# url-kaist/Quatro

Measured on NVIDIA H100. Metric: registrations/sec (64-ring pair), higher is better.
Workload: dtype f32 (front end, match, graph filter) / f64 (graph boundary, GNC, COTE)

## Files before the change

### quatro_b200/csrc/frontend.cu

```cuda
#include <cub/device/device_radix_sort.cuh>
#include <type_traits>

#include "fpfh_math.cuh"
#include "handle.cuh"

namespace qb {

size_t sort_temp_bytes(int max_items) {
  size_t bytes = 0;
  cub::DeviceRadixSort::SortPairs(nullptr, bytes, (const uint64_t*)nullptr, (uint64_t*)nullptr, (const uint32_t*)nullptr,
                                  (uint32_t*)nullptr, max_items, 0, 64, (cudaStream_t)0);
  return bytes;
}

int sort_pairs(Lane* h, int n_items, int end_bit) {
  if (n_items <= 0) return QB200_OK;
  size_t bytes = h->cub_bytes;
  QB_CUDA_TRY(h, cub::DeviceRadixSort::SortPairs(h->cub_temp.get(), bytes, h->key_a.get(), h->key_b.get(), h->val_a.get(), h->val_b.get(), n_items, 0, end_bit,
                                                 h->stream));
  h->launches += 1 + (end_bit + 7) / 8;
  return QB200_OK;
}

static int clog2(int n) {
  int b = 0;
  while ((1 << b) < n) ++b;
  return b;
}


__global__ void __launch_bounds__(256) voxel_bbox_kernel(const float4* const* __restrict__ cloud_ptr, const int* __restrict__ cloud_n,
                                                         const CloudFront* __restrict__ front, int* __restrict__ bbox,
                                                         int* __restrict__ n_valid, int* __restrict__ chunk_cnt) {
  const int cloud = blockIdx.y;
  const int n = cloud_n[cloud];
  const int skip_flagged = front[cloud].skip_flagged;
  const float4* __restrict__ pts = cloud_ptr[cloud];
  int mn0 = INT_MAX, mn1 = INT_MAX, mn2 = INT_MAX, mx0 = INT_MIN, mx1 = INT_MIN, mx2 = INT_MIN, cnt = 0;
  constexpr int kInFlight = 8;
  __shared__ int s_cc[kVsChunks];
  if (threadIdx.x < kVsChunks) s_cc[threadIdx.x] = 0;
  __syncthreads();
  const int cs = vox_chunk_size(n);
  const int per_cta = kVsChunks / gridDim.x;
  for (int cl = 0; cl < per_cta; ++cl) {
    const int ch = blockIdx.x * per_cta + cl;
    const int c0 = ch * cs, c1 = min(n, c0 + cs);
    int ccnt = 0;
    for (int i0 = c0 + threadIdx.x; i0 < c1; i0 += kInFlight * 256) {
      float4 pp[kInFlight];
#pragma unroll
      for (int j = 0; j < kInFlight; ++j) pp[j] = i0 + j * 256 < c1 ? __ldg(pts + i0 + j * 256) : make_float4(NAN, NAN, NAN, 0.f);
#pragma unroll
      for (int j = 0; j < kInFlight; ++j) {
        const float4 p = pp[j];
        if (i0 + j * 256 >= c1 || !raw_point_kept(p, skip_flagged)) continue;
        const int ox = float_ordered(p.x), oy = float_ordered(p.y), oz = float_ordered(p.z);
        mn0 = min(mn0, ox); mn1 = min(mn1, oy); mn2 = min(mn2, oz);
        mx0 = max(mx0, ox); mx1 = max(mx1, oy); mx2 = max(mx2, oz);
        ++ccnt;
      }
    }
    cnt += ccnt;
    ccnt = __reduce_add_sync(0xffffffffu, ccnt);
    if (lane_id() == 0 && ccnt) atomicAdd(&s_cc[ch], ccnt);
  }
  __syncthreads();
  if ((int)threadIdx.x < per_cta) chunk_cnt[cloud * kVsChunks + blockIdx.x * per_cta + threadIdx.x] = s_cc[blockIdx.x * per_cta + threadIdx.x];
#pragma unroll
  for (int o = 16; o > 0; o >>= 1) {
    mn0 = min(mn0, __shfl_xor_sync(0xffffffffu, mn0, o)); mn1 = min(mn1, __shfl_xor_sync(0xffffffffu, mn1, o));
    mn2 = min(mn2, __shfl_xor_sync(0xffffffffu, mn2, o)); mx0 = max(mx0, __shfl_xor_sync(0xffffffffu, mx0, o));
    mx1 = max(mx1, __shfl_xor_sync(0xffffffffu, mx1, o)); mx2 = max(mx2, __shfl_xor_sync(0xffffffffu, mx2, o));
    cnt += __shfl_xor_sync(0xffffffffu, cnt, o);
  }
  __shared__ int s_red[7];
  if (threadIdx.x == 0) { s_red[0] = s_red[1] = s_red[2] = INT_MAX; s_red[3] = s_red[4] = s_red[5] = INT_MIN; s_red[6] = 0; }
  __syncthreads();
  if (lane_id() == 0 && cnt) {
    atomicMin(&s_red[0], mn0); atomicMin(&s_red[1], mn1); atomicMin(&s_red[2], mn2);
    atomicMax(&s_red[3], mx0); atomicMax(&s_red[4], mx1); atomicMax(&s_red[5], mx2);
    atomicAdd(&s_red[6], cnt);
  }
  __syncthreads();
  if (threadIdx.x == 0 && s_red[6]) {
    int* b = bbox + cloud * 6;
    atomicMin(b + 0, s_red[0]); atomicMin(b + 1, s_red[1]); atomicMin(b + 2, s_red[2]);
    atomicMax(b + 3, s_red[3]); atomicMax(b + 4, s_red[4]); atomicMax(b + 5, s_red[5]);
    atomicAdd(n_valid + cloud, s_red[6]);
  }
}

__global__ void __launch_bounds__(1024) run_heads_kernel(int mode, const uint64_t* keys, const uint64_t* keys_b, const int* __restrict__ seg_off,
                                                         int V, int key_shift, const CloudFront* __restrict__ front, const int* __restrict__ bbox,
                                                         const int* __restrict__ n_valid_in, int* __restrict__ starts,
                                                         uint64_t* __restrict__ cell_keys, int* __restrict__ n_out, int* __restrict__ n_valid_out,
                                                         int* __restrict__ cloud_status, int* __restrict__ digits_out) {
  __shared__ int sm[33];
  __shared__ int s_overflow, s_valid;
  const int cloud = blockIdx.x;
  const int off = mode == 0 ? seg_off[cloud] : cloud * V;
  const int n = mode == 0 ? n_valid_in[cloud] : V;
  const int digits = mode == 0 ? vox_digits(bbox + cloud * 6, n, front[cloud].inv_leaf) : 0;
  if (digits & 1) keys = keys_b;
  if (threadIdx.x == 0) {
    s_overflow = digits < 0 ? 1 : 0;
    s_valid = 0;
    if (digits_out) digits_out[cloud] = digits;
  }
  __syncthreads();
  if (s_overflow) {
    if (threadIdx.x == 0) {
      n_out[cloud] = 0;
      cloud_status[cloud] = QB200_ERR_VOXEL_OVERFLOW;
      starts[(size_t)cloud * (V + 1)] = 0;
    }
    return;
  }
  int carry = 0;
  constexpr int kPer = 4;
  for (int base = 0; base < n; base += kPer * blockDim.x) {
    const int p0 = base + kPer * threadIdx.x;
    uint64_t k[kPer];
    bool valid[kPer];
    int head[kPer], nh = 0, nv = 0;
    uint64_t kprev = (p0 > 0 && p0 < n) ? keys[off + p0 - 1] >> key_shift : 0;
#pragma unroll
    for (int j = 0; j < kPer; ++j) {
      const int p = p0 + j;
      k[j] = 0; valid[j] = false; head[j] = 0;
      if (p < n) {
        k[j] = keys[off + p] >> key_shift;
        valid[j] = mode == 0 ? (k[j] & kVoxMask) != kVoxInvalid : (k[j] & kCellMask) != kCellInvalid;
        head[j] = (valid[j] && (p == 0 || k[j] != kprev)) ? 1 : 0;
        kprev = k[j];
      }
      nh += head[j]; nv += valid[j] ? 1 : 0;
    }
    int both;
    const int exb = block_excl_scan(nh | (nv << 16), sm, &both);
    int rank = carry + (exb & 0xFFFF);
    const int tot = both & 0xFFFF, vtot = both >> 16;
#pragma unroll
    for (int j = 0; j < kPer; ++j) {
      if (head[j]) {
        if (rank <= V) {
          starts[(size_t)cloud * (V + 1) + rank] = p0 + j;
          if (mode == 1 && rank < V) cell_keys[(size_t)cloud * V + rank] = k[j] & kCellMask;
        }
        ++rank;
      }
    }
    carry += tot;
    if (threadIdx.x == 0) s_valid += vtot;
  }
  if (threadIdx.x == 0) {
    const int valid_total = s_valid;
    int nv = carry;
    if (nv > V) {
      nv = V;
      cloud_status[cloud] = QB200_CAPACITY_EXCEEDED;
    } else {
      starts[(size_t)cloud * (V + 1) + nv] = valid_total;
    }
    n_out[cloud] = nv;
    if (n_valid_out) n_valid_out[cloud] = valid_total;
  }
}

__global__ void __launch_bounds__(128) voxel_centroid_kernel(const float4* const* __restrict__ cloud_ptr, const int* __restrict__ raw_off,
                                                             const uint64_t* sorted_keys, const uint64_t* keys_b, const int* __restrict__ vox_digits,
                                                             uint64_t idx_mask,
                                                             const int* __restrict__ starts, const int* __restrict__ n_vox, int V,
                                                             float4* __restrict__ vox_pts) {
  const int cloud = blockIdx.y;
  const int r = blockIdx.x * blockDim.x + threadIdx.x;
  if (r >= n_vox[cloud]) return;
  const uint64_t* __restrict__ keys = ((vox_digits[cloud] & 1) ? keys_b : sorted_keys) + raw_off[cloud];
  const float4* __restrict__ pts = cloud_ptr[cloud];
  const int a = starts[(size_t)cloud * (V + 1) + r], b = starts[(size_t)cloud * (V + 1) + r + 1];
  float sx = 0.f, sy = 0.f, sz = 0.f;
  int t = a;
  for (; t + 4 <= b; t += 4) {
    const uint64_t k0 = keys[t], k1 = keys[t + 1], k2 = keys[t + 2], k3 = keys[t + 3];
    const float4 p0 = __ldg(pts + (k0 & idx_mask)), p1 = __ldg(pts + (k1 & idx_mask)), p2 = __ldg(pts + (k2 & idx_mask)),
                 p3 = __ldg(pts + (k3 & idx_mask));
    sx += p0.x; sy += p0.y; sz += p0.z;
    sx += p1.x; sy += p1.y; sz += p1.z;
    sx += p2.x; sy += p2.y; sz += p2.z;
    sx += p3.x; sy += p3.y; sz += p3.z;
  }
  for (; t < b; ++t) {
    const float4 p = __ldg(pts + (keys[t] & idx_mask));
    sx += p.x; sy += p.y; sz += p.z;
  }
  const float cnt = (float)(b - a);
  vox_pts[(size_t)cloud * V + r] = make_float4(sx / cnt, sy / cnt, sz / cnt, 1.0f);
}

__global__ void __launch_bounds__(256) lattice_keys_kernel(const float4* __restrict__ pts, const int* __restrict__ n_pts, int V,
                                                           const CloudFront* __restrict__ front, uint64_t* __restrict__ keys,
                                                           uint32_t* __restrict__ vals) {
  const int cloud = blockIdx.y;
  const int r = blockIdx.x * blockDim.x + threadIdx.x;
  if (r >= V) return;
  uint64_t cell = kCellInvalid;
  if (r < n_pts[cloud]) {
    const float inv_cell = front[cloud].inv_cell;
    const float4 p = pts[(size_t)cloud * V + r];
    if (isfinite(p.x) && isfinite(p.y) && isfinite(p.z)) {
      const int ci = (int)floorf(p.x * inv_cell), cj = (int)floorf(p.y * inv_cell), ck = (int)floorf(p.z * inv_cell);
      if (cell_ok(ci, cj, ck)) cell = cell_key(ci, cj, ck);
    }
  }
  keys[(size_t)cloud * V + r] = ((uint64_t)cloud << kCloudShift) | cell;
  vals[(size_t)cloud * V + r] = (uint32_t)r;
}

struct LatticeView {
  const float4* pts;
  const uint64_t* ckeys;
  const int* cstart;
  const uint32_t* order;
  int n_cells;
  float inv;
};

template <class R2, class F>
__device__ __forceinline__ void walk_cells(const LatticeView& L, const float4 pq, const R2& r2_src, int c0, int c1, F&& f) {
  if (c0 >= c1) return;
  const float r2 = r2_src;
  const int t1 = L.cstart[c1];
  for (int t = L.cstart[c0]; t < t1; t += 4) {
    int p[4];
    float4 pp[4];
#pragma unroll
    for (int e = 0; e < 4; ++e) p[e] = t + e < t1 ? (int)L.order[t + e] : -1;
#pragma unroll
    for (int e = 0; e < 4; ++e) pp[e] = p[e] >= 0 ? L.pts[p[e]] : make_float4(0.f, 0.f, 0.f, 0.f);
#pragma unroll
    for (int e = 0; e < 4; ++e) {
      if (p[e] < 0) continue;
      const float dx = pq.x - pp[e].x, dy = pq.y - pp[e].y, dz = pq.z - pp[e].z;
      const float d2 = (dx * dx + dy * dy) + dz * dz;
      if (d2 < r2) f(p[e], d2, pp[e]);
    }
  }
}

template <bool kLockstep = true, class R2, class F>
__device__ __forceinline__ void for_each_neighbor(const LatticeView& L, const float4 pq, int m, const R2& r2, F&& f) {
  if (!(isfinite(pq.x) && isfinite(pq.y) && isfinite(pq.z))) return;
  const int ci = (int)floorf(pq.x * L.inv), cj = (int)floorf(pq.y * L.inv), ck = (int)floorf(pq.z * L.inv);
  if (!cell_ok(ci, cj, ck)) return;
  const int ilo = max(ci - m, -kOffIJ), ihi = min(ci + m, kOffIJ - 2);
  if (kLockstep && m == 1) {
    uint64_t lo[9], hi[9];
    int a[9], b[9], e[9];
#pragma unroll
    for (int r = 0; r < 9; ++r) {
      const int k = ck + r / 3 - 1, j = cj + r % 3 - 1;
      const bool ok = !(k < -kOffK || k >= kOffK - 1 || j < -kOffIJ || j >= kOffIJ - 1);
      lo[r] = ok ? cell_key(ilo, j, k) : 1;
      hi[r] = ok ? cell_key(ihi, j, k) : 0;
      a[r] = 0; b[r] = ok ? L.n_cells : 0;
      e[r] = 0;
    }
    const int steps = 33 - __clz(L.n_cells | 1);
    for (int s = 0; s < steps; ++s) {
#pragma unroll
      for (int r = 0; r < 9; ++r) {
        if (a[r] < b[r]) {
          const int mid = (a[r] + b[r]) >> 1;
          if (L.ckeys[mid] < lo[r]) a[r] = mid + 1; else b[r] = mid;
        }
      }
    }
#pragma unroll
    for (int r = 0; r < 9; ++r) {
      int c = a[r];
#pragma unroll
      for (int q = 0; q < 3; ++q)
        if (c < L.n_cells && hi[r] >= lo[r] && L.ckeys[c] <= hi[r]) ++c;
      e[r] = c;
    }
#pragma unroll
    for (int r = 0; r < 9; ++r) walk_cells(L, pq, r2, a[r], e[r], f);
    return;
  }
  for (int dk = -m; dk <= m; ++dk) {
    const int k = ck + dk;
    if (k < -kOffK || k >= kOffK - 1) continue;
    for (int dj = -m; dj <= m; ++dj) {
      const int j = cj + dj;
      if (j < -kOffIJ || j >= kOffIJ - 1) continue;
      const uint64_t lo = cell_key(ilo, j, k), hi = cell_key(ihi, j, k);
      int a = 0, b = L.n_cells;
      while (a < b) {
        const int mid = (a + b) >> 1;
        if (L.ckeys[mid] < lo) a = mid + 1; else b = mid;
      }
      int c = a;
      while (c < L.n_cells && L.ckeys[c] <= hi) ++c;
      walk_cells(L, pq, r2, a, c, f);
    }
  }
}

__device__ __forceinline__ LatticeView make_view(int cloud, int V, const float4* pts, const uint64_t* cell_key, const int* cell_start,
                                                 const uint32_t* order, const int* n_cells, float inv) {
  LatticeView L;
  L.pts = pts + (size_t)cloud * V;
  L.ckeys = cell_key + (size_t)cloud * V;
  L.cstart = cell_start + (size_t)cloud * (V + 1);
  L.order = order + (size_t)cloud * V;
  L.n_cells = n_cells[cloud];
  L.inv = inv;
  return L;
}

constexpr int kNbrThreads = 128;
constexpr int kNbrCap = 32;

struct WalkPos {
  int row = 0;
  int t = -1;
};

__device__ __forceinline__ int walk_chunk(const LatticeView& L, const float4 pq, int m, float r2, WalkPos& pos,
                                          uint32_t (*nbr)[kNbrThreads]) {
  const int w = 2 * m + 1;
  if (!(isfinite(pq.x) && isfinite(pq.y) && isfinite(pq.z))) { pos.row = w * w; return 0; }
  const int ci = (int)floorf(pq.x * L.inv), cj = (int)floorf(pq.y * L.inv), ck = (int)floorf(pq.z * L.inv);
  if (!cell_ok(ci, cj, ck)) { pos.row = w * w; return 0; }
  const int ilo = max(ci - m, -kOffIJ), ihi = min(ci + m, kOffIJ - 2);
  int n = 0;
  for (; pos.row < w * w; ++pos.row, pos.t = -1) {
    const int k = ck + pos.row / w - m, j = cj + pos.row % w - m;
    if (k < -kOffK || k >= kOffK - 1 || j < -kOffIJ || j >= kOffIJ - 1) continue;
    const uint64_t lo = cell_key(ilo, j, k), hi = cell_key(ihi, j, k);
    int a = 0, b = L.n_cells;
    while (a < b) {
      const int mid = (a + b) >> 1;
      if (L.ckeys[mid] < lo) a = mid + 1; else b = mid;
    }
    int c = a;
    while (c < L.n_cells && L.ckeys[c] <= hi) ++c;
    if (a >= c) continue;
    const int t1 = L.cstart[c];
    for (int t = pos.t >= 0 ? pos.t : L.cstart[a]; t < t1; ++t) {
      const int p = (int)L.order[t];
      const float4 pp = L.pts[p];
      const float dx = pq.x - pp.x, dy = pq.y - pp.y, dz = pq.z - pp.z;
      const float d2 = (dx * dx + dy * dy) + dz * dz;
      if (!(d2 < r2)) continue;
      if (n == kNbrCap) { pos.t = t; return n; }
      nbr[n++][threadIdx.x] = (uint32_t)p;
    }
  }
  return n;
}

__global__ void __launch_bounds__(kNbrThreads) nbr_list_kernel(const float4* __restrict__ pts, const int* __restrict__ n_pts, int V,
                                                               const uint64_t* __restrict__ cell_key, const int* __restrict__ cell_start,
                                                               const uint32_t* __restrict__ order, const int* __restrict__ n_cells,
                                                               const CloudFront* __restrict__ front, uint32_t* __restrict__ nbr_list,
                                                               int* __restrict__ nbr_cnt) {
  volatile __shared__ float s_r2;
  const int cloud = blockIdx.y;
  if (threadIdx.x == 0) s_r2 = front[cloud].rf2;
  __syncthreads();
  const int q = blockIdx.x * blockDim.x + threadIdx.x;
  if (q >= n_pts[cloud]) return;
  const int m = front[cloud].mf;
  const LatticeView L = make_view(cloud, V, pts, cell_key, cell_start, order, n_cells, front[cloud].inv_cell);
  uint32_t* __restrict__ gl = nbr_list + (size_t)cloud * kNbrGlobalCap * V + q;
  int k = 0;
  for_each_neighbor(L, L.pts[q], m, s_r2, [&](int p, float, const float4) {
    if (k < kNbrGlobalCap) gl[(size_t)k * V] = (uint32_t)p;
    ++k;
  });
  nbr_cnt[(size_t)cloud * V + q] = k;
}

__global__ void __launch_bounds__(128) normals_kernel(const float4* __restrict__ pts, const int* __restrict__ n_pts, int V,
                                                      const uint64_t* __restrict__ cell_key, const int* __restrict__ cell_start,
                                                      const uint32_t* __restrict__ order, const int* __restrict__ n_cells,
                                                      const CloudFront* __restrict__ front, const uint32_t* __restrict__ nbr_list,
                                                      const int* __restrict__ nbr_cnt, float4* __restrict__ normals) {
  volatile __shared__ float s_r2;
  const int cloud = blockIdx.y;
  if (threadIdx.x == 0) s_r2 = front[cloud].rn2;
  __syncthreads();
  const int q = blockIdx.x * blockDim.x + threadIdx.x;
  if (q >= n_pts[cloud]) return;
  const float4* __restrict__ P = pts + (size_t)cloud * V;
  const float4 pq = P[q];
  float accu[9] = {0.f, 0.f, 0.f, 0.f, 0.f, 0.f, 0.f, 0.f, 0.f};
  int cnt = 0;
  auto add = [&](const float4 pp) {
    accu[0] += pp.x * pp.x; accu[1] += pp.x * pp.y; accu[2] += pp.x * pp.z;
    accu[3] += pp.y * pp.y; accu[4] += pp.y * pp.z; accu[5] += pp.z * pp.z;
    accu[6] += pp.x; accu[7] += pp.y; accu[8] += pp.z;
    ++cnt;
  };
  const int kq = nbr_cnt[(size_t)cloud * V + q];
  if (front[cloud].list_usable && kq <= kNbrGlobalCap) {
    const uint32_t* __restrict__ gl = nbr_list + (size_t)cloud * kNbrGlobalCap * V + q;
    const float r2 = s_r2;
    for (int t = 0; t < kq; ++t) {
      const float4 pp = P[gl[(size_t)t * V]];
      const float dx = pq.x - pp.x, dy = pq.y - pp.y, dz = pq.z - pp.z;
      const float d2 = (dx * dx + dy * dy) + dz * dz;
      if (d2 < r2) add(pp);
    }
  } else {
    const LatticeView L = make_view(cloud, V, pts, cell_key, cell_start, order, n_cells, front[cloud].inv_cell);
    for_each_neighbor(L, pq, front[cloud].mn, s_r2, [&](int, float, const float4 pp) { add(pp); });
  }
  float out[4];
  qb_normal_from_accu(accu, cnt, pq.x, pq.y, pq.z, out);
  normals[(size_t)cloud * V + q] = make_float4(out[0], out[1], out[2], out[3]);
}

constexpr int kSpfhThreads = kNbrThreads;
static_assert(kNbrGlobalCap < 65536, "spfh_kernel<false> counts in 16 bits");
__device__ __forceinline__ int spfh_slot(int b) { return b + b / 11; }
template <bool kRare>
__global__ void __launch_bounds__(kSpfhThreads) spfh_kernel(const float4* __restrict__ pts, const float4* __restrict__ normals,
                                                            const int* __restrict__ n_pts, int V, const uint64_t* __restrict__ cell_key,
                                                            const int* __restrict__ cell_start, const uint32_t* __restrict__ order,
                                                            const int* __restrict__ n_cells, const CloudFront* __restrict__ front,
                                                            float* __restrict__ spfh, const uint32_t* __restrict__ nbr_list,
                                                            const int* __restrict__ nbr_cnt) {
  using Count = typename std::conditional<kRare, unsigned, unsigned short>::type;
  __shared__ Count cnts[kDescDim][kSpfhThreads];
  __shared__ uint32_t nbr[kRare ? kNbrCap : 1][kNbrThreads];
  const int cloud = blockIdx.y;
  const int q = blockIdx.x * blockDim.x + threadIdx.x;
  if (q >= n_pts[cloud]) return;
  int k = nbr_cnt[(size_t)cloud * V + q];
  if ((k > kNbrGlobalCap) != kRare) return;
  const LatticeView L = make_view(cloud, V, pts, cell_key, cell_start, order, n_cells, front[cloud].inv_cell);
  const float4* __restrict__ nrm = normals + (size_t)cloud * V;
  const float4 pq = L.pts[q];
  const float4 nq = nrm[q];
#pragma unroll
  for (int b = 0; b < kDescDim; ++b) cnts[b][threadIdx.x] = 0;
  auto feature = [&](int p) {
    if (p == q) return;
    const float4 pp = L.pts[p];
    const float4 np = nrm[p];
    float f1, f2, f3;
    if (!qb_pair_features(pq.x, pq.y, pq.z, nq.x, nq.y, nq.z, pp.x, pp.y, pp.z, np.x, np.y, np.z, &f1, &f2, &f3)) return;
    int b1, b2, b3;
    qb_feature_bins(f1, f2, f3, &b1, &b2, &b3);
    cnts[b1][threadIdx.x]++;
    cnts[11 + b2][threadIdx.x]++;
    cnts[22 + b3][threadIdx.x]++;
  };
  if (!kRare) {
    const uint32_t* __restrict__ gl = nbr_list + (size_t)cloud * kNbrGlobalCap * V + q;
    for (int t = 0; t < k; ++t) feature((int)gl[(size_t)t * V]);
  } else {
    k = 0;
    WalkPos pos;
    const int m = front[cloud].mf;
    const float r2 = front[cloud].rf2;
    const int rows = (2 * m + 1) * (2 * m + 1);
    while (pos.row < rows) {
      const int n = walk_chunk(L, pq, m, r2, pos, nbr);
      for (int t = 0; t < n; ++t) feature((int)nbr[t][threadIdx.x]);
      k += n;
    }
  }
  float* __restrict__ out = spfh + ((size_t)cloud * V + q) * kDescPad;
  const float incr = k >= 2 ? 100.0f / (float)(k - 1) : 0.0f;
  for (int b = 0; b < kDescDim; ++b) {
    const int c = (int)cnts[b][threadIdx.x];
    float v = 0.0f;
    for (int t = 0; t < c; ++t) v += incr;
    out[spfh_slot(b)] = v;
  }
  out[11] = 0.0f; out[23] = 0.0f; out[35] = 0.0f;
}

__global__ void __launch_bounds__(3 * kNbrThreads, 3) fpfh_list_kernel(const float4* __restrict__ pts, const int* __restrict__ n_pts, int V,
                                                                    const float* __restrict__ spfh, const uint32_t* __restrict__ nbr_list,
                                                                    const int* __restrict__ nbr_cnt, float* __restrict__ desc_t) {
  const int cloud = blockIdx.y;
  const int third = threadIdx.x / kNbrThreads;
  const int q = blockIdx.x * kNbrThreads + (threadIdx.x - third * kNbrThreads);
  if (q >= n_pts[cloud]) return;
  const int kq = nbr_cnt[(size_t)cloud * V + q];
  if (kq > kNbrGlobalCap) return;
  const float4* __restrict__ P = pts + (size_t)cloud * V;
  const float4* __restrict__ sp = reinterpret_cast<const float4*>(spfh + (size_t)cloud * V * kDescPad) + 3 * third;
  const float4 pq = P[q];
  float o[11];
#pragma unroll
  for (int b = 0; b < 11; ++b) o[b] = 0.0f;
  double sum = 0.0;
  const uint32_t* __restrict__ gl = nbr_list + (size_t)cloud * kNbrGlobalCap * V + q;
  int p_n = kq > 0 ? (int)gl[0] : 0;
  int p_nn = kq > 1 ? (int)gl[(size_t)V] : 0;
  float4 pp_n = P[p_n];
  float4 a0 = __ldg(sp + (size_t)p_n * (kDescPad / 4)), a1 = __ldg(sp + (size_t)p_n * (kDescPad / 4) + 1), a2 = __ldg(sp + (size_t)p_n * (kDescPad / 4) + 2);
  for (int t = 0; t < kq; ++t) {
    const float4 pp = pp_n, t0 = a0, t1 = a1, t2 = a2;
    if (t + 1 < kq) {
      const int pn = p_nn;
      if (t + 2 < kq) p_nn = (int)gl[(size_t)(t + 2) * V];
      pp_n = P[pn];
      a0 = __ldg(sp + (size_t)pn * (kDescPad / 4)); a1 = __ldg(sp + (size_t)pn * (kDescPad / 4) + 1); a2 = __ldg(sp + (size_t)pn * (kDescPad / 4) + 2);
    }
    const float dx = pq.x - pp.x, dy = pq.y - pp.y, dz = pq.z - pp.z;
    const float d2 = (dx * dx + dy * dy) + dz * dz;
    if (d2 == 0.0f) continue;
    const float weight = 1.0f / d2;
    const float sv[11] = {t0.x, t0.y, t0.z, t0.w, t1.x, t1.y, t1.z, t1.w, t2.x, t2.y, t2.z};
#pragma unroll
    for (int b = 0; b < 11; ++b) { const float v = sv[b] * weight; sum += v; o[b] += v; }
  }
  if (sum != 0.0) sum = 100.0 / sum;
  const float g = (float)sum;
  float* __restrict__ out = desc_t + (size_t)cloud * kDescK * V + (size_t)(11 * third) * V + q;
#pragma unroll
  for (int b = 0; b < 11; ++b) out[(size_t)b * V] = o[b] * g;
}

__global__ void __launch_bounds__(kNbrThreads) fpfh_rare_kernel(const float4* __restrict__ pts, const int* __restrict__ n_pts, int V,
                                                                const uint64_t* __restrict__ cell_key, const int* __restrict__ cell_start,
                                                                const uint32_t* __restrict__ order, const int* __restrict__ n_cells,
                                                                const CloudFront* __restrict__ front, const float* __restrict__ spfh,
                                                                const int* __restrict__ nbr_cnt, float* __restrict__ desc_t) {
  const int cloud = blockIdx.y;
  const int q = blockIdx.x * blockDim.x + threadIdx.x;
  if (q >= n_pts[cloud]) return;
  if (nbr_cnt[(size_t)cloud * V + q] <= kNbrGlobalCap) return;
  const int m = front[cloud].mf;
  const float r2 = front[cloud].rf2;
  const LatticeView L = make_view(cloud, V, pts, cell_key, cell_start, order, n_cells, front[cloud].inv_cell);
  const float4* __restrict__ sp = reinterpret_cast<const float4*>(spfh + (size_t)cloud * V * kDescPad);
  const float4 pq = L.pts[q];
  float o[kDescDim];
#pragma unroll
  for (int b = 0; b < kDescDim; ++b) o[b] = 0.0f;
  double s0 = 0.0, s1 = 0.0, s2 = 0.0;
  for_each_neighbor<false>(L, pq, m, r2, [&](int p, float d2, const float4) {
    if (d2 == 0.0f) return;
    const float weight = 1.0f / d2;
    float s[kDescPad];
#pragma unroll
    for (int v4 = 0; v4 < kDescPad / 4; ++v4) {
      const float4 t = __ldg(sp + (size_t)p * (kDescPad / 4) + v4);
      s[4 * v4] = t.x; s[4 * v4 + 1] = t.y; s[4 * v4 + 2] = t.z; s[4 * v4 + 3] = t.w;
    }
#pragma unroll
    for (int b = 0; b < 11; ++b) { const float v = s[b] * weight; s0 += v; o[b] += v; }
#pragma unroll
    for (int b = 0; b < 11; ++b) { const float v = s[12 + b] * weight; s1 += v; o[11 + b] += v; }
#pragma unroll
    for (int b = 0; b < 11; ++b) { const float v = s[24 + b] * weight; s2 += v; o[22 + b] += v; }
  });
  if (s0 != 0.0) s0 = 100.0 / s0;
  if (s1 != 0.0) s1 = 100.0 / s1;
  if (s2 != 0.0) s2 = 100.0 / s2;
  const float g0 = (float)s0, g1 = (float)s1, g2 = (float)s2;
  float* __restrict__ out = desc_t + (size_t)cloud * kDescK * V + q;
#pragma unroll
  for (int b = 0; b < 11; ++b) out[(size_t)b * V] = o[b] * g0;
#pragma unroll
  for (int b = 11; b < 22; ++b) out[(size_t)b * V] = o[b] * g1;
#pragma unroll
  for (int b = 22; b < 33; ++b) out[(size_t)b * V] = o[b] * g2;
}

constexpr int kExportTile = 128, kExportThreads = 256;

__global__ void __launch_bounds__(kExportThreads) feature_export_kernel(ExportSrc s, int V, ExportDst d) {
  __shared__ float tile[kExportTile * kDescDim];
  const int cloud = blockIdx.y, q0 = blockIdx.x * kExportTile, tid = threadIdx.x;
  const int st = s.status ? s.status[cloud] : QB200_OK;
  const int n = st == QB200_OK ? s.n[cloud] : 0;
  if (blockIdx.x == 0 && tid == 0) {
    if (d.counts) d.counts[cloud] = n;
    if (d.status) d.status[cloud] = st;
  }
  const int m_all = min(n, d.cap);
  if (q0 >= m_all) return;
  const int m = min(kExportTile, m_all - q0);
  const size_t from = (size_t)cloud * V + q0, to = (size_t)cloud * d.stride + q0;
  for (int i = tid; i < m; i += kExportThreads) {
    if (d.vox) d.vox[to + i] = __ldg(s.vox + from + i);
    if (d.nrm) d.nrm[to + i] = __ldg(s.nrm + from + i);
  }
  if (!d.desc) return;
  const float* __restrict__ col = s.desc + (size_t)cloud * kDescK * V + q0;
  for (int i = tid; i < kDescDim * kExportTile; i += kExportThreads) {
    const int dim = i / kExportTile, q = i % kExportTile;
    if (q < m) tile[q * kDescDim + dim] = __ldg(col + (size_t)dim * V + q);
  }
  __syncthreads();
  float* __restrict__ out = d.desc + to * kDescDim;
  for (int i = tid; i < m * kDescDim; i += kExportThreads) out[i] = tile[i];
}

constexpr int kImportTile = 128, kImportThreads = 256;

__global__ void __launch_bounds__(kImportThreads) feature_import_kernel(const FeatureSrc* __restrict__ table, int V, float4* __restrict__ vox_pts,
                                                                        float* __restrict__ desc_t, int* __restrict__ n_vox) {
  __shared__ float tile[kImportTile * kDescDim];
  const int cloud = blockIdx.y, q0 = blockIdx.x * kImportTile, tid = threadIdx.x;
  const FeatureSrc f = table[cloud];
  if (blockIdx.x == 0 && tid == 0) n_vox[cloud] = f.n;
  if (q0 >= f.n) return;
  const int m = min(kImportTile, f.n - q0);
  if (f.pts)
    for (int i = tid; i < m; i += kImportThreads) vox_pts[(size_t)cloud * V + q0 + i] = __ldg(f.pts + q0 + i);
  if (!f.desc) return;
  const float* __restrict__ src = f.desc + (size_t)q0 * kDescDim;
  for (int i = tid; i < m * kDescDim; i += kImportThreads) tile[i] = __ldg(src + i);
  __syncthreads();
  float* __restrict__ out = desc_t + (size_t)cloud * kDescK * V + q0;
  for (int i = tid; i < kDescDim * kImportTile; i += kImportThreads) {
    const int d = i / kImportTile, q = i % kImportTile;
    if (q < m) out[(size_t)d * V + q] = tile[q * kDescDim + d];
  }
}

void front_voxel(CloudFront* e, float leaf, int skip_flagged) {
  e->inv_leaf = 1.0f / leaf;
  e->skip_flagged = skip_flagged;
}

void front_lattice(CloudFront* e, float normal_radius, float fpfh_radius, float cell) {
  e->inv_cell = 1.0f / cell;
  e->mn = (int)ceilf(normal_radius * e->inv_cell + 1e-3f);
  e->mf = (int)ceilf(fpfh_radius * e->inv_cell + 1e-3f);
  e->rn2 = (float)((double)normal_radius * (double)normal_radius);
  e->rf2 = (float)((double)fpfh_radius * (double)fpfh_radius);
  e->list_usable = (e->mn <= e->mf && e->rn2 <= e->rf2) ? 1 : 0;
}

int upload_front(Lane* L, int n) {
  QB_CUDA_TRY(L, cudaMemcpyAsync(L->d_front, L->h_front, (size_t)n * sizeof(CloudFront), cudaMemcpyHostToDevice, L->stream));
  return QB200_OK;
}

int launch_voxel(Lane* h, int n_clouds) {
  if (n_clouds <= 0) return QB200_OK;
  const dim3 gb(n_clouds >= 16 ? 16 : 64, n_clouds);
  int* chunk_cnt = reinterpret_cast<int*>(h->val_b.get());
  voxel_bbox_kernel<<<gb, 256, 0, h->stream>>>(h->d_cloud_ptr, h->d_cloud_n, h->d_front, h->ctr.bbox, h->ctr.n_valid, chunk_cnt);
  h->launches += 1;
  const int idx_bits = clog2(h->R > 2 ? h->R : 2);
  if (int rc = launch_voxel_sort(h, n_clouds, idx_bits)) return rc;
  run_heads_kernel<<<n_clouds, 1024, 0, h->stream>>>(0, h->key_a, h->key_b, h->d_raw_off, h->V, idx_bits, h->d_front, h->ctr.bbox, h->ctr.n_valid,
                                                     h->vox_start, nullptr, h->ctr.n_vox, nullptr, h->ctr.cloud_status, h->ctr.vox_digits);
  const dim3 gc((h->V + 127) / 128, n_clouds);
  voxel_centroid_kernel<<<gc, 128, 0, h->stream>>>(h->d_cloud_ptr, h->d_raw_off, h->key_a, h->key_b, h->ctr.vox_digits,
                                                   (1ull << idx_bits) - 1, h->vox_start, h->ctr.n_vox, h->V, h->vox_pts);
  h->launches += 2;
  QB_CUDA_TRY(h, cudaGetLastError());
  return QB200_OK;
}

int launch_fpfh(Lane* h, int n_clouds) {
  if (n_clouds <= 0) return QB200_OK;
  const int V = h->V;
  const dim3 gl((V + 255) / 256, n_clouds);
  lattice_keys_kernel<<<gl, 256, 0, h->stream>>>(h->vox_pts, h->ctr.n_vox, V, h->d_front, h->key_a, h->val_a);
  h->launches++;
  int rc = launch_cloud_sort(h, n_clouds, h->ctr.n_vox, 18, 36);
  if (rc == QB200_ERR_UNSUPPORTED) rc = sort_pairs(h, n_clouds * V, kCloudShift + clog2(n_clouds > 1 ? n_clouds : 2));
  if (rc) return rc;
  run_heads_kernel<<<n_clouds, 1024, 0, h->stream>>>(1, h->key_b, nullptr, nullptr, V, 0, nullptr, nullptr, nullptr, h->cell_start, h->cell_key,
                                                     h->ctr.n_cells, h->ctr.n_lat, h->ctr.cloud_status, nullptr);
  const dim3 gp((V + 127) / 128, n_clouds);
  nbr_list_kernel<<<gp, kNbrThreads, 0, h->stream>>>(h->vox_pts, h->ctr.n_vox, V, h->cell_key, h->cell_start, h->val_b, h->ctr.n_cells,
                                                     h->d_front, h->nbr_list, h->nbr_cnt);
  normals_kernel<<<gp, 128, 0, h->stream>>>(h->vox_pts, h->ctr.n_vox, V, h->cell_key, h->cell_start, h->val_b, h->ctr.n_cells, h->d_front,
                                            h->nbr_list, h->nbr_cnt, h->normals);
  spfh_kernel<false><<<gp, kSpfhThreads, 0, h->stream>>>(h->vox_pts, h->normals, h->ctr.n_vox, V, h->cell_key, h->cell_start, h->val_b,
                                                         h->ctr.n_cells, h->d_front, h->spfh, h->nbr_list, h->nbr_cnt);
  spfh_kernel<true><<<gp, kSpfhThreads, 0, h->stream>>>(h->vox_pts, h->normals, h->ctr.n_vox, V, h->cell_key, h->cell_start, h->val_b,
                                                        h->ctr.n_cells, h->d_front, h->spfh, h->nbr_list, h->nbr_cnt);
  fpfh_list_kernel<<<gp, 3 * kNbrThreads, 0, h->stream>>>(h->vox_pts, h->ctr.n_vox, V, h->spfh, h->nbr_list, h->nbr_cnt, h->desc_t);
  fpfh_rare_kernel<<<gp, kNbrThreads, 0, h->stream>>>(h->vox_pts, h->ctr.n_vox, V, h->cell_key, h->cell_start, h->val_b, h->ctr.n_cells,
                                                      h->d_front, h->spfh, h->nbr_cnt, h->desc_t);
  h->launches += 3;
  h->launches += 4;
  QB_CUDA_TRY(h, cudaGetLastError());
  return QB200_OK;
}

int launch_feature_export(Lane* h, int n_clouds, const ExportSrc& src, const ExportDst& dst, int max_n) {
  if (n_clouds <= 0) return QB200_OK;
  const int m = max_n < dst.cap ? max_n : dst.cap;
  const dim3 g(((m > 1 ? m : 1) + kExportTile - 1) / kExportTile, n_clouds);
  feature_export_kernel<<<g, kExportThreads, 0, h->stream>>>(src, h->V, dst);
  h->launches++;
  QB_CUDA_TRY(h, cudaGetLastError());
  return QB200_OK;
}

int export_desc_rows(Lane* h, const float* desc, const int* n, int m) {
  ExportSrc s{nullptr, nullptr, desc, n, nullptr};
  ExportDst d{nullptr, nullptr, h->aos_scratch, m, m, nullptr, nullptr};
  return launch_feature_export(h, 1, s, d, m);
}

ExportDst ExportDst::caller(const qb200_feature_out& o, long long first) {
  const long long c = o.cap_per_scan;
  ExportDst d;
  d.vox = o.vox4 ? reinterpret_cast<float4*>(o.vox4) + first * c : nullptr;
  d.nrm = o.normals4 ? reinterpret_cast<float4*>(o.normals4) + first * c : nullptr;
  d.desc = o.desc33 ? o.desc33 + first * c * kDescDim : nullptr;
  d.stride = c;
  d.cap = o.cap_per_scan;
  d.counts = d.status = nullptr;
  return d;
}

size_t ExportDst::carve(unsigned char* base, int n, int cap, const qb200_feature_out& o, ExportDst* d) {
  const size_t k = (size_t)n * cap;
  size_t off = 0;
  auto take = [&](size_t bytes, bool want) -> unsigned char* {
    if (!want) return nullptr;
    unsigned char* p = base ? base + off : nullptr;
    off += (bytes + 15) & ~(size_t)15;
    return p;
  };
  d->counts = reinterpret_cast<int*>(take((size_t)n * sizeof(int), true));
  d->status = reinterpret_cast<int*>(take((size_t)n * sizeof(int), true));
  d->vox = reinterpret_cast<float4*>(take(k * sizeof(float4), o.vox4));
  d->nrm = reinterpret_cast<float4*>(take(k * sizeof(float4), o.normals4));
  d->desc = reinterpret_cast<float*>(take(k * kDescDim * sizeof(float), o.desc33));
  d->stride = cap;
  d->cap = cap;
  return off;
}
int launch_feature_import(Lane* h, int n_clouds) {
  if (n_clouds <= 0) return QB200_OK;
  int n_max = 1;
  for (int c = 0; c < n_clouds; ++c) n_max = h->h_feat[c].n > n_max ? h->h_feat[c].n : n_max;
  const dim3 g((n_max + kImportTile - 1) / kImportTile, n_clouds);
  feature_import_kernel<<<g, kImportThreads, 0, h->stream>>>(h->d_feat, h->V, h->vox_pts, h->desc_t, h->ctr.n_vox);
  h->launches++;
  QB_CUDA_TRY(h, cudaGetLastError());
  return QB200_OK;
}

}
```

Baseline: 13570.

## Process query points in lattice-sorted order across front-end neighbor kernels

Threads now map to slots in the cell-sorted order rather than to the original point index, so neighbouring threads in a warp query spatially adjacent points. This is meant to make the cell walks and neighbour gathers more coherent, lowering divergence and improving cache hits. The neighbour list and count arrays are indexed by sorted slot, while normals, SPFH and descriptors are still written at the original index. The cost is one extra indirection load per thread and scattered output writes.

```diff
diff --git a/quatro_b200/csrc/frontend.cu b/quatro_b200/csrc/frontend.cu
--- a/quatro_b200/csrc/frontend.cu
+++ b/quatro_b200/csrc/frontend.cu
@@ -370,17 +370,18 @@
   const int cloud = blockIdx.y;
   if (threadIdx.x == 0) s_r2 = front[cloud].rf2;
   __syncthreads();
-  const int q = blockIdx.x * blockDim.x + threadIdx.x;
-  if (q >= n_pts[cloud]) return;
+  const int s = blockIdx.x * blockDim.x + threadIdx.x;
+  if (s >= n_pts[cloud]) return;
   const int m = front[cloud].mf;
   const LatticeView L = make_view(cloud, V, pts, cell_key, cell_start, order, n_cells, front[cloud].inv_cell);
-  uint32_t* __restrict__ gl = nbr_list + (size_t)cloud * kNbrGlobalCap * V + q;
+  const int q = (int)L.order[s];
+  uint32_t* __restrict__ gl = nbr_list + (size_t)cloud * kNbrGlobalCap * V + s;
   int k = 0;
   for_each_neighbor(L, L.pts[q], m, s_r2, [&](int p, float, const float4) {
     if (k < kNbrGlobalCap) gl[(size_t)k * V] = (uint32_t)p;
     ++k;
   });
-  nbr_cnt[(size_t)cloud * V + q] = k;
+  nbr_cnt[(size_t)cloud * V + s] = k;
 }
 
 __global__ void __launch_bounds__(128) normals_kernel(const float4* __restrict__ pts, const int* __restrict__ n_pts, int V,
@@ -392,9 +393,10 @@
   const int cloud = blockIdx.y;
   if (threadIdx.x == 0) s_r2 = front[cloud].rn2;
   __syncthreads();
-  const int q = blockIdx.x * blockDim.x + threadIdx.x;
-  if (q >= n_pts[cloud]) return;
+  const int s = blockIdx.x * blockDim.x + threadIdx.x;
+  if (s >= n_pts[cloud]) return;
   const float4* __restrict__ P = pts + (size_t)cloud * V;
+  const int q = (int)order[(size_t)cloud * V + s];
   const float4 pq = P[q];
   float accu[9] = {0.f, 0.f, 0.f, 0.f, 0.f, 0.f, 0.f, 0.f, 0.f};
   int cnt = 0;
@@ -404,9 +406,9 @@
     accu[6] += pp.x; accu[7] += pp.y; accu[8] += pp.z;
     ++cnt;
   };
-  const int kq = nbr_cnt[(size_t)cloud * V + q];
+  const int kq = nbr_cnt[(size_t)cloud * V + s];
   if (front[cloud].list_usable && kq <= kNbrGlobalCap) {
-    const uint32_t* __restrict__ gl = nbr_list + (size_t)cloud * kNbrGlobalCap * V + q;
+    const uint32_t* __restrict__ gl = nbr_list + (size_t)cloud * kNbrGlobalCap * V + s;
     const float r2 = s_r2;
     for (int t = 0; t < kq; ++t) {
       const float4 pp = P[gl[(size_t)t * V]];
@@ -420,7 +422,7 @@
   }
   float out[4];
   qb_normal_from_accu(accu, cnt, pq.x, pq.y, pq.z, out);
-  normals[(size_t)cloud * V + q] = make_float4(out[0], out[1], out[2], out[3]);
+  normals[(size_t)cloud * V + __ldcg(order + (size_t)cloud * V + s)] = make_float4(out[0], out[1], out[2], out[3]);
 }
 
 constexpr int kSpfhThreads = kNbrThreads;
@@ -437,11 +439,12 @@
   __shared__ Count cnts[kDescDim][kSpfhThreads];
   __shared__ uint32_t nbr[kRare ? kNbrCap : 1][kNbrThreads];
   const int cloud = blockIdx.y;
-  const int q = blockIdx.x * blockDim.x + threadIdx.x;
-  if (q >= n_pts[cloud]) return;
-  int k = nbr_cnt[(size_t)cloud * V + q];
+  const int s = blockIdx.x * blockDim.x + threadIdx.x;
+  if (s >= n_pts[cloud]) return;
+  int k = nbr_cnt[(size_t)cloud * V + s];
   if ((k > kNbrGlobalCap) != kRare) return;
   const LatticeView L = make_view(cloud, V, pts, cell_key, cell_start, order, n_cells, front[cloud].inv_cell);
+  const int q = (int)L.order[s];
   const float4* __restrict__ nrm = normals + (size_t)cloud * V;
   const float4 pq = L.pts[q];
   const float4 nq = nrm[q];
@@ -460,7 +463,7 @@
     cnts[22 + b3][threadIdx.x]++;
   };
   if (!kRare) {
-    const uint32_t* __restrict__ gl = nbr_list + (size_t)cloud * kNbrGlobalCap * V + q;
+    const uint32_t* __restrict__ gl = nbr_list + (size_t)cloud * kNbrGlobalCap * V + s;
     for (int t = 0; t < k; ++t) feature((int)gl[(size_t)t * V]);
   } else {
     k = 0;
@@ -486,22 +489,23 @@
 }
 
 __global__ void __launch_bounds__(3 * kNbrThreads, 3) fpfh_list_kernel(const float4* __restrict__ pts, const int* __restrict__ n_pts, int V,
-                                                                    const float* __restrict__ spfh, const uint32_t* __restrict__ nbr_list,
-                                                                    const int* __restrict__ nbr_cnt, float* __restrict__ desc_t) {
+                                                                    const uint32_t* __restrict__ order, const float* __restrict__ spfh,
+                                                                    const uint32_t* __restrict__ nbr_list, const int* __restrict__ nbr_cnt,
+                                                                    float* __restrict__ desc_t) {
   const int cloud = blockIdx.y;
   const int third = threadIdx.x / kNbrThreads;
-  const int q = blockIdx.x * kNbrThreads + (threadIdx.x - third * kNbrThreads);
-  if (q >= n_pts[cloud]) return;
-  const int kq = nbr_cnt[(size_t)cloud * V + q];
+  const int s = blockIdx.x * kNbrThreads + (threadIdx.x - third * kNbrThreads);
+  if (s >= n_pts[cloud]) return;
+  const int kq = nbr_cnt[(size_t)cloud * V + s];
   if (kq > kNbrGlobalCap) return;
   const float4* __restrict__ P = pts + (size_t)cloud * V;
   const float4* __restrict__ sp = reinterpret_cast<const float4*>(spfh + (size_t)cloud * V * kDescPad) + 3 * third;
-  const float4 pq = P[q];
+  const float4 pq = P[order[(size_t)cloud * V + s]];
   float o[11];
 #pragma unroll
   for (int b = 0; b < 11; ++b) o[b] = 0.0f;
   double sum = 0.0;
-  const uint32_t* __restrict__ gl = nbr_list + (size_t)cloud * kNbrGlobalCap * V + q;
+  const uint32_t* __restrict__ gl = nbr_list + (size_t)cloud * kNbrGlobalCap * V + s;
   int p_n = kq > 0 ? (int)gl[0] : 0;
   int p_nn = kq > 1 ? (int)gl[(size_t)V] : 0;
   float4 pp_n = P[p_n];
@@ -524,7 +528,7 @@
   }
   if (sum != 0.0) sum = 100.0 / sum;
   const float g = (float)sum;
-  float* __restrict__ out = desc_t + (size_t)cloud * kDescK * V + (size_t)(11 * third) * V + q;
+  float* __restrict__ out = desc_t + (size_t)cloud * kDescK * V + (size_t)(11 * third) * V + __ldcg(order + (size_t)cloud * V + s);
 #pragma unroll
   for (int b = 0; b < 11; ++b) out[(size_t)b * V] = o[b] * g;
 }
@@ -535,12 +539,13 @@
                                                                 const CloudFront* __restrict__ front, const float* __restrict__ spfh,
                                                                 const int* __restrict__ nbr_cnt, float* __restrict__ desc_t) {
   const int cloud = blockIdx.y;
-  const int q = blockIdx.x * blockDim.x + threadIdx.x;
-  if (q >= n_pts[cloud]) return;
-  if (nbr_cnt[(size_t)cloud * V + q] <= kNbrGlobalCap) return;
+  const int s = blockIdx.x * blockDim.x + threadIdx.x;
+  if (s >= n_pts[cloud]) return;
+  if (nbr_cnt[(size_t)cloud * V + s] <= kNbrGlobalCap) return;
   const int m = front[cloud].mf;
   const float r2 = front[cloud].rf2;
   const LatticeView L = make_view(cloud, V, pts, cell_key, cell_start, order, n_cells, front[cloud].inv_cell);
+  const int q = (int)L.order[s];
   const float4* __restrict__ sp = reinterpret_cast<const float4*>(spfh + (size_t)cloud * V * kDescPad);
   const float4 pq = L.pts[q];
   float o[kDescDim];
@@ -686,7 +691,7 @@
                                                          h->ctr.n_cells, h->d_front, h->spfh, h->nbr_list, h->nbr_cnt);
   spfh_kernel<true><<<gp, kSpfhThreads, 0, h->stream>>>(h->vox_pts, h->normals, h->ctr.n_vox, V, h->cell_key, h->cell_start, h->val_b,
                                                         h->ctr.n_cells, h->d_front, h->spfh, h->nbr_list, h->nbr_cnt);
-  fpfh_list_kernel<<<gp, 3 * kNbrThreads, 0, h->stream>>>(h->vox_pts, h->ctr.n_vox, V, h->spfh, h->nbr_list, h->nbr_cnt, h->desc_t);
+  fpfh_list_kernel<<<gp, 3 * kNbrThreads, 0, h->stream>>>(h->vox_pts, h->ctr.n_vox, V, h->val_b, h->spfh, h->nbr_list, h->nbr_cnt, h->desc_t);
   fpfh_rare_kernel<<<gp, kNbrThreads, 0, h->stream>>>(h->vox_pts, h->ctr.n_vox, V, h->cell_key, h->cell_start, h->val_b, h->ctr.n_cells,
                                                       h->d_front, h->spfh, h->nbr_cnt, h->desc_t);
   h->launches += 3;
```

New measurement: 13790, median of 6. 1.02x the previous value.
